# OCR-D/ocrd_keraslm

Measured on AMD Instinct MI355X. Metric: chars/sec training (stacked-LSTM forward+backward+Adam), higher is better.
Workload: dtype bf16; 1 GPU; cfg2: depth=2 width=512 length=256 V=256 1 context, stateful training, 3072 streams/GPU, synthetic 10M-char corpus (SURVEY.md 8d); streams_per_gpu=3072, global_batch=3072, seq_len=256, parallelism=dp1

## Files before the change

### include/keraslm_hip.h

```cpp
#ifndef KERASLM_HIP_H
#define KERASLM_HIP_H

#include <stddef.h>
#include <stdint.h>

#ifdef __cplusplus
extern "C" {
#endif

#define KL_ABI_VERSION 1

enum {
  KL_OK = 0,
  KL_ERR_SHAPE = 1,
  KL_ERR_LAUNCH = 2,
  KL_ERR_STATE = 3,
  KL_ERR_WORKSPACE = 4,
  KL_ERR_ARG = 5
};

#define KL_PREC_BF16 1
#define KL_PREC_SPLIT 3

typedef struct kl_config {
  int32_t depth;
  int32_t width;
  int32_t voc_size;
  int32_t n_ctx;
  int32_t ctx_vocab;
  int32_t ctx_dim;
} kl_config;

typedef struct kl_handle kl_handle;

int kl_abi_version(void);
const char* kl_error_string(int code);

size_t kl_param_count(const kl_config* cfg);
int kl_param_layout(const kl_config* cfg, int index, char* name, size_t name_cap, size_t* offset, size_t* rows,
                    size_t* cols);

kl_handle* kl_create(const kl_config* cfg);
void kl_destroy(kl_handle* h);

size_t kl_derived_bytes(const kl_handle* h);
int kl_bind(kl_handle* h, float* params , void* derived , size_t derived_bytes);

int kl_prepare(kl_handle* h, int precision, void* stream);

size_t kl_window_workspace_bytes(const kl_handle* h, int B, int T, int training);

int kl_set_window_mode(kl_handle* h, int last_only);

int kl_set_loss_rows(kl_handle* h, int rows);

int kl_forward_window(kl_handle* h, int B, int T, const int32_t* idx, const int32_t* ctx, const int32_t* tgt,
                      float* states, float* probs, float* loss_acc, void* ws, size_t ws_bytes, void* stream);

int kl_train_window(kl_handle* h, int B, int T, const int32_t* idx, const int32_t* ctx, const int32_t* tgt,
                    float* states, const float* dropout_masks, float* grads, float* loss_acc, void* ws,
                    size_t ws_bytes, void* stream);

int kl_adam_step(kl_handle* h, const float* grads, float* m, float* v, int t, float lr, float b1, float b2,
                 float eps, float clip, void* stream);
int kl_adam_step_scaled(kl_handle* h, const float* grads, float grad_scale, float* m, float* v, int t, float lr,
                        float b1, float b2, float eps, float clip, void* stream);

size_t kl_step_workspace_bytes(const kl_handle* h, int n);
int kl_step_batch(kl_handle* h, int n, const int32_t* idx, const int32_t* ctx, float* pool, const int32_t* slot_in,
                  const int32_t* slot_out, float* probs, void* ws, size_t ws_bytes, void* stream);

void* kl_host_alloc(size_t bytes);
void kl_host_free(void* p);
size_t kl_step_host_workspace_bytes(const kl_handle* h, int n);
int kl_step_batch_host(kl_handle* h, int n, const int32_t* idx, const int32_t* ctx, const int32_t* slot_in,
                       const int32_t* slot_out, const int32_t* target, float* pool, int head_k, float* probs_host,
                       float* heads_host, uint32_t* done_host, uint32_t ticket, void* ws, size_t ws_bytes, void* stream);
int kl_step_wait(const uint32_t* done_host, uint32_t ticket, double timeout_s);

int kl_state_dist2(const kl_handle* h, int n, const float* pool, const int32_t* a, const int32_t* b, int k,
                   float* out, void* stream);

int kl_trace_enable(kl_handle* h, int on);
int kl_trace_read(kl_handle* h, int kind, int* n_launches, float* total_ms, int* persistent,
                  double* flops_per_launch);
const char* kl_trace_kernel_name(kl_handle* h, int kind);

int kl_test_gemm_tn(const uint16_t* A, const uint16_t* B, void* C, const float* bias, int M, int N, int K, long lda,
                    long ldb, long ldc, int out_mode, int splits, void* stream);
int kl_test_gemm_an(const uint16_t* A_km, const uint16_t* B, float* C, int M, int N, int K, long lda_km, long ldb,
                    long ldc, int c_transposed, int b_km, void* stream);
int kl_test_thin_gemm(const float* A, long lda, const uint16_t* WT_hi, const uint16_t* WT_lo, long ldw, int M, int N,
                      int K, float* C, long ldc, int split, void* stream);

#ifdef __cplusplus
}
#endif
#endif
```

### ocrd_keraslm_amd/csrc/api.hip

```cpp
#include <hip/hip_runtime.h>
#include <stdio.h>
#include <stdlib.h>
#include <string.h>
#include <time.h>

#include <functional>
#include <utility>

#include <vector>

#include "kl_common.h"
#include "kl_kernels.h"

namespace {

inline size_t align_up(size_t x, size_t a) { return (x + a - 1) / a * a; }
inline int round_up_i(int x, int a) { return (x + a - 1) / a * a; }

struct Carver {
  unsigned char* base;
  size_t off = 0;
  explicit Carver(void* b) : base(reinterpret_cast<unsigned char*>(b)) {}
  template <typename T>
  T* take(size_t count) {
// ... 1749 lines not shown
    int e = 0;
    for (int l = 0; l < L && e == 0; ++l) {
      KlIncCellArgs a;
      memset(&a, 0, sizeof(a));
      a.n = n; a.W = W; a.split = split;
      a.pool = pool; a.slot_ld = slot_ld;
      a.h_off = 2 * l * W; a.c_off = (2 * l + 1) * W; a.x_off = l > 0 ? 2 * (l - 1) * W : -1;
      a.UF = d.UF[l]; a.KF = d.KF[l];
      a.bias = P + h->off_b[l];
      if (l == 0) {
        a.T1 = d.EK; a.i1 = dev_idx; a.T2 = d.CtxK[0]; a.i2 = dev_idx;
      }
      e = kl_launch_inc_cell(a, s, &hx, l == 0 ? dev_idx : nullptr);
      if (e == KL_ERR_SHAPE && l > 0) return e;
    }
    if (e == 0) {
      KlOperand op;
      memset(&op, 0, sizeof(op));
      op.A = pool + (size_t)2 * (L - 1) * W; op.lda = slot_ld; op.row_index = dev_idx; op.a_is_f32 = 1;
      op.WT_hi = d.E_hi; op.WT_lo = split == 3 ? d.E_lo : nullptr; op.ldw = W; op.K = W;
      KL_TRY(kl_launch_thin_gemm(&op, n, V, logits, V, nullptr, split, s));
      f.softmax = 1; f.slot_out = dev_idx;
      return kl_launch_step_finish(f, target ? &tx : nullptr, s);
    }
    if (e != KL_ERR_SHAPE) return e;
  }
  {
    const int Cc = C > 0 ? C : 1;
    std::vector<int32_t>& pk = h->host_pack;
    pk.resize((size_t)n * (4 + Cc));
    memcpy(pk.data(), idx, (size_t)n * 4);
    memcpy(pk.data() + n, slot_in, (size_t)n * 4);
    memcpy(pk.data() + 2 * (size_t)n, slot_out, (size_t)n * 4);
    if (target) memcpy(pk.data() + 3 * (size_t)n, target, (size_t)n * 4);
    else memset(pk.data() + 3 * (size_t)n, 0, (size_t)n * 4);
    if (C > 0) memcpy(pk.data() + 4 * (size_t)n, ctx, (size_t)n * C * 4);
    if (hipMemcpyAsync(dev_idx, pk.data(), pk.size() * 4, hipMemcpyHostToDevice, s) != hipSuccess) return KL_ERR_LAUNCH;
    KL_TRY(kl_step_batch(h, n, dev_idx, C > 0 ? dev_idx + 4 * (size_t)n : nullptr, pool, dev_idx + n, dev_idx + 2 * (size_t)n, logits,
                         rest, rest_bytes, stream));
    f.softmax = 0; f.slot_out = dev_idx + 2 * (size_t)n;
    f.target = target ? dev_idx + 3 * (size_t)n : nullptr;
    return kl_launch_step_finish(f, nullptr, s);
  }
}

int kl_step_wait(const uint32_t* done_host, uint32_t ticket, double timeout_s) {
  if (!done_host) return KL_ERR_ARG;
  const volatile uint32_t* flag = done_host;
  struct timespec t0;
  clock_gettime(CLOCK_MONOTONIC, &t0);
  for (unsigned spins = 0;; ++spins) {
    if (__atomic_load_n(flag, __ATOMIC_ACQUIRE) == ticket) return 0;
    __builtin_ia32_pause();
    if ((spins & 0x3ff) == 0x3ff) {
      struct timespec t1;
      clock_gettime(CLOCK_MONOTONIC, &t1);
      if ((double)(t1.tv_sec - t0.tv_sec) + 1e-9 * (double)(t1.tv_nsec - t0.tv_nsec) > timeout_s) {
        return hipGetLastError() == hipSuccess ? KL_ERR_STATE : KL_ERR_LAUNCH;
      }
    }
  }
}

int kl_state_dist2(const kl_handle* h, int n, const float* pool, const int32_t* a, const int32_t* b, int k, float* out,
                   void* stream) {
  if (!h || !pool || !a || !b || !out || n < 1) return KL_ERR_ARG;
  if (k < 0 || k >= 2 * h->cfg.depth) return KL_ERR_ARG;
  const int W = h->cfg.width;
  hipLaunchKernelGGL(state_dist2_kernel, dim3((n + 3) / 4), dim3(256), 0, (hipStream_t)stream, pool,
                     (long)2 * h->cfg.depth * W, W, k, a, b, n, out);
  return hip_ok(hipGetLastError());
}

int kl_test_gemm_tn(const uint16_t* A, const uint16_t* B, void* C, const float* bias, int M, int N, int K, long lda,
                    long ldb, long ldc, int out_mode, int splits, void* stream) {
  return kl_launch_gemm_tn(A, B, C, bias, M, N, K, lda, ldb, ldc, out_mode, splits, 1.f, (hipStream_t)stream);
}

int kl_test_gemm_an(const uint16_t* A_km, const uint16_t* B, float* C, int M, int N, int K, long lda_km, long ldb,
                    long ldc, int c_transposed, int b_km, void* stream) {
  return kl_launch_gemm_an(A_km, B, C, M, N, K, lda_km, ldb, ldc, c_transposed, (hipStream_t)stream, b_km);
}

int kl_test_thin_gemm(const float* A, long lda, const uint16_t* WT_hi, const uint16_t* WT_lo, long ldw, int M, int N,
                      int K, float* C, long ldc, int split, void* stream) {
  KlOperand op;
  memset(&op, 0, sizeof(op));
  op.A = A; op.lda = lda; op.a_is_f32 = 1; op.WT_hi = WT_hi; op.WT_lo = WT_lo; op.ldw = ldw; op.K = K;
  return kl_launch_thin_gemm(&op, M, N, C, ldc, nullptr, split, (hipStream_t)stream);
}

}

extern "C" int kl_test_fwd_step(const uint16_t* A, long lda, const uint16_t* WT, long ldw, int K, int n_ops,
                                int n_rows, int W, int fused, int iters, float* c_out, uint16_t* h_out,
                                void* stream) {
  KlFwdStep st[4];
  if (fused < 1 || fused > 4 || n_ops < 1 || n_ops > 2) return KL_ERR_ARG;
  for (int f = 0; f < fused; ++f) {
    KlFwdStep& S = st[f];
    memset(&S, 0, sizeof(S));
    S.n_rows = n_rows; S.W = W; S.split = 1; S.n_ops = n_ops;
    for (int p = 0; p < n_ops; ++p) {
      KlOperand& o = S.op[p];
      o.A = A; o.lda = lda; o.WT_hi = WT + (size_t)(f * 2 + p) * (size_t)4 * W * ldw; o.ldw = ldw;
      o.K = K; o.a_is_f32 = 0;
    }
    S.c_out = c_out + (size_t)f * n_rows * W; S.c_out_ld = W;
    S.h_out_bf16 = h_out + (size_t)f * n_rows * W; S.h_out_bf16_ld = W;
  }
  for (int i = 0; i < iters; ++i) {
    int e = kl_launch_fwd_steps(st, fused, (hipStream_t)stream);
    if (e) return e;
  }
  return 0;
}


namespace {

int run_graphed(kl_handle* h, const kl_handle::GraphKey& key, hipStream_t s, const std::function<int()>& body) {
  if (!h->graphs_enabled || h->trace_on || s == nullptr) return body();
  for (auto& g : h->graphs)
    if (g.first == key) return hip_ok(hipGraphLaunch(g.second, s));
  if (hipStreamBeginCapture(s, hipStreamCaptureModeThreadLocal) != hipSuccess) {
    (void)hipGetLastError();
    h->graphs_enabled = false;
    return body();
  }
  const int e = body();
  hipGraph_t graph = nullptr;
  const hipError_t ce = hipStreamEndCapture(s, &graph);
  if (e != 0 || ce != hipSuccess || graph == nullptr) {
    if (graph) (void)hipGraphDestroy(graph);
    (void)hipGetLastError();
    h->graphs_enabled = false;
    return e != 0 ? e : body();
  }
  hipGraphExec_t exec = nullptr;
  const hipError_t ie = hipGraphInstantiate(&exec, graph, nullptr, nullptr, 0);
  (void)hipGraphDestroy(graph);
  if (ie != hipSuccess || exec == nullptr) {
    (void)hipGetLastError();
    h->graphs_enabled = false;
    return body();
  }
  if (h->graphs.size() >= 16) h->drop_graphs();
  h->graphs.emplace_back(key, exec);
  return hip_ok(hipGraphLaunch(exec, s));
}

}

extern "C" int kl_set_loss_rows(kl_handle* h, int rows) {
  if (!h || rows < 0) return KL_ERR_ARG;
  h->loss_rows = rows;
  return 0;
}

extern "C" int kl_set_window_mode(kl_handle* h, int last_only) {
  if (!h) return KL_ERR_ARG;
  h->last_only = last_only ? 1 : 0;
  return 0;
}

extern "C" int kl_forward_window(kl_handle* h, int B, int T, const int32_t* idx, const int32_t* ctx, const int32_t* tgt,
// ... 83 lines not shown
```

### ocrd_keraslm_amd/csrc/gemm.hip

```cpp
#include <stdlib.h>
#include <string.h>

#include "kl_common.h"
#include "kl_kernels.h"

namespace {

constexpr int BN = 128, BK = 64;
constexpr int NTHREADS = 256;

__device__ __forceinline__ int lds_off(int row, int chunk) {
  return row * 128 + ((chunk ^ ((row >> 1) & 7)) << 4);
}

template <int OUT, int BM>
__global__ __launch_bounds__(NTHREADS) void gemm_tn_kernel(
    const bf16_t* __restrict__ A, const bf16_t* __restrict__ B, void* __restrict__ Cv,
    const float* __restrict__ bias, int M, int N, int K, long lda, long ldb, long ldc,
    int k_per_split, float alpha) {
  constexpr int WM = BM / 64;
  constexpr int WN = 4 / WM;
  constexpr int NT = BN / WN / 16;
  constexpr int ALOADS = BM * 8 / NTHREADS;
  extern __shared__ __attribute__((aligned(16))) unsigned char smem[];
// ... 574 lines not shown
        fa[i].u = *reinterpret_cast<const uint4*>(a_base + lds_off(wm * WROWS + i * 16 + fr, s * 4 + fq));
#pragma unroll
      for (int j = 0; j < NT; ++j)
        fb[j].u = *reinterpret_cast<const uint4*>(b_base + lds_off(wn * WCOLS + j * 16 + fr, s * 4 + fq));
      if (more) issue_half(nstage, s);
      __builtin_amdgcn_s_setprio(1);
#pragma unroll
      for (int i = 0; i < RF; ++i)
#pragma unroll
        for (int j = 0; j < NT; ++j) acc[i][j] = mfma16(fa[i].v, fb[j].v, acc[i][j]);
      __builtin_amdgcn_s_setprio(0);
    }
    stage = stage + 1 < LSTAGES ? stage + 1 : 0;
    if (++kt_c == nkt) {
      const int L = first + it_c * (int)gridDim.x;
      const int m0 = (L / tiles_n) * TBM, n0 = (L % tiles_n) * LBN;
      const int esz = out_bf16 ? 2 : 4;
      const long bytes = ((long)(M - m0 - 1) * ldc + (N - n0)) * esz;
      const __amdgpu_buffer_rsrc_t rsC = __builtin_amdgcn_make_buffer_rsrc(
          reinterpret_cast<char*>(C) + ((long)m0 * ldc + n0) * esz, 0, (int)(unsigned)(bytes > 0xffffffffL ? 0xffffffffL : bytes), 0x00020000);
      const int k = fr & 3, c4 = fr & ~3;
#pragma unroll
      for (int i = 0; i < RF; ++i) {
#pragma unroll
        for (int j = 0; j < NT; ++j) {
          f32x4 v = acc[i][j];
          quad_transpose(v, k);
          const int row = wm * WROWS + i * 16 + fq * 4 + k;
          const int col = wn * WCOLS + j * 16 + c4;
          f32x4 bv = f32x4{0.f, 0.f, 0.f, 0.f};
          if (bias != nullptr && n0 + col + 3 < N) bv = *reinterpret_cast<const f32x4*>(bias_l + n0 + col);
          v = v * alpha + bv;
          const unsigned off = (n0 + col < N) ? (unsigned)(((long)row * ldc + col) * esz) : 0xfffffff0u;
          if (out_bf16) {
            typedef __attribute__((ext_vector_type(2))) unsigned int u32x2g;
            const u32x2g pk = u32x2g{(unsigned)f2bf(v[0]) | ((unsigned)f2bf(v[1]) << 16), (unsigned)f2bf(v[2]) | ((unsigned)f2bf(v[3]) << 16)};
            __builtin_amdgcn_raw_buffer_store_b64(pk, rsC, (int)off, 0, 0);
          } else {
            __builtin_amdgcn_raw_buffer_store_b128(__builtin_bit_cast(u32x4g, v), rsC, (int)off, 0, 0);
          }
          acc[i][j] = f32x4{0.f, 0.f, 0.f, 0.f};
        }
      }
      kt_c = 0;
      ++it_c;
      stored = 2;
    }
  }
}

template <int RF, int WM, int WN>
int launch_long_t(int out_mode, dim3 grid, hipStream_t stream, const bf16_t* A, const bf16_t* B, void* C, const float* bias,
                  int M, int N, int K, long lda, long ldb, long ldc, int k_per_split, float alpha,
                  const KlGateEpi* gate = nullptr) {
  KlGateEpi epi;
  if (gate) epi = *gate;
  else memset(&epi, 0, sizeof(epi));
  const size_t lds = (size_t)LSTAGES * (16 * RF * WM + LBN) * 128;
  static const bool ilv = !(getenv("KL_GEMM_ILV") && getenv("KL_GEMM_ILV")[0] == '0');
  static const int remap = !(getenv("KL_GEMM_XCD") && getenv("KL_GEMM_XCD")[0] == '0');
#define KL_LONG_CASE(O)                                                                                                  \
  do {                                                                                                                   \
    static KlLdsGrant grant_a, grant_b;                                                  \
    if (kl_grant_lds(grant_a, reinterpret_cast<const void*>(&gemm_tn_long_kernel<O, true, RF, WM, WN>), lds)) return KL_ERR_LAUNCH;  \
    if (kl_grant_lds(grant_b, reinterpret_cast<const void*>(&gemm_tn_long_kernel<O, false, RF, WM, WN>), lds)) return KL_ERR_LAUNCH; \
    if (ilv) hipLaunchKernelGGL((gemm_tn_long_kernel<O, true, RF, WM, WN>), grid, dim3(64 * WM * WN), lds, stream, A, B, C,  \
                                bias, M, N, K, lda, ldb, ldc, k_per_split, alpha, epi, remap, 0, KlGemmSecond{});                        \
    else hipLaunchKernelGGL((gemm_tn_long_kernel<O, false, RF, WM, WN>), grid, dim3(64 * WM * WN), lds, stream, A, B, C,     \
                            bias, M, N, K, lda, ldb, ldc, k_per_split, alpha, epi, remap, 0, KlGemmSecond{});                            \
  } while (0)
  if (out_mode == 0) KL_LONG_CASE(0);
  else if (out_mode == 1) KL_LONG_CASE(1);
  else if (out_mode == 3) KL_LONG_CASE(3);
  else KL_LONG_CASE(2);
#undef KL_LONG_CASE
  return 0;
}

int launch_long(int out_mode, dim3 grid, hipStream_t stream, const bf16_t* A, const bf16_t* B, void* C, const float* bias,
                int M, int N, int K, long lda, long ldb, long ldc, int k_per_split, float alpha) {
  return launch_long_t<4, 4, 2>(out_mode, grid, stream, A, B, C, bias, M, N, K, lda, ldb, ldc, k_per_split, alpha);
}

}

int kl_launch_gemm_tn(const bf16_t* A, const bf16_t* B, void* C, const float* bias, int M, int N, int K,
                      long lda, long ldb, long ldc, int out_mode, int splits, float alpha, hipStream_t stream) {
  if (M <= 0 || N <= 0 || K <= 0) return 0;
  if ((K & 7) || (lda & 7) || (ldb & 7)) return KL_ERR_SHAPE;
  if (splits < 1) splits = 1;
  if (out_mode != 2) splits = 1;
  static const int long_mode = getenv("KL_GEMM_LONG") ? atoi(getenv("KL_GEMM_LONG")) : 2;
  const bool long_ok = (K % BK) == 0 && lda < (1L << 22) && ldb < (1L << 22);
  if (long_mode >= 1 && long_ok && out_mode == 2 && K >= 8192) {
    const int tiles = ((M + LBM - 1) / LBM) * ((N + LBN - 1) / LBN);
    int sp = (256 + tiles - 1) / tiles;
    const int nk = K / BK;
    if (sp > nk / 16) sp = nk / 16;
    if (sp < 1) sp = 1;
    const int kps = ((nk + sp - 1) / sp) * BK;
    sp = (K + kps - 1) / kps;
    dim3 grid((N + LBN - 1) / LBN, (M + LBM - 1) / LBM, sp);
    const int e = launch_long(out_mode, grid, stream, A, B, C, bias, M, N, K, lda, ldb, ldc, kps, alpha);
    if (e != 0) return e;
    return hipGetLastError() == hipSuccess ? 0 : KL_ERR_LAUNCH;
  }
  static const bool small_all = getenv("KL_GEMM_SMALL_ALL") && getenv("KL_GEMM_SMALL_ALL")[0] == '1';
  static const bool pers = !(getenv("KL_GEMM_PERS") && getenv("KL_GEMM_PERS")[0] == '0');
  if (pers && !small_all && long_mode >= 2 && long_ok && (out_mode == 0 || out_mode == 1) && K >= 6 * BK && K <= 16 * BK && (N & 3) == 0 && (ldc & 3) == 0 &&
      ((size_t)C & 15) == 0 && (bias == nullptr || N <= 2048) &&
      (long)((M + LBM - 1) / LBM) * ((N + LBN - 1) / LBN) >= 512) {
    static int n_wg = 0;
    if (!n_wg) {
      int dev = 0;
      hipDeviceProp_t prop;
      n_wg = (hipGetDevice(&dev) == hipSuccess && hipGetDeviceProperties(&prop, dev) == hipSuccess && prop.multiProcessorCount >= 8)
                 ? (prop.multiProcessorCount & ~7) : 256;
    }
    const int tiles_n = (N + LBN - 1) / LBN, total = ((M + LBM - 1) / LBM) * tiles_n;
    const size_t lds = (size_t)LSTAGES * (LBM + LBN) * 128 + (bias ? (size_t)N * 4 : 0);
    static KlLdsGrant grant;
    if (kl_grant_lds(grant, reinterpret_cast<const void*>(&gemm_tn_pers_kernel), (size_t)LSTAGES * (LBM + LBN) * 128 + 2048 * 4)) return KL_ERR_LAUNCH;
    hipLaunchKernelGGL(gemm_tn_pers_kernel, dim3(n_wg), dim3(512), lds, stream, A, B, (float*)C, bias, M, N, K, lda, ldb, ldc,
                       alpha, tiles_n, total, out_mode == 1 ? 1 : 0);
    return hipGetLastError() == hipSuccess ? 0 : KL_ERR_LAUNCH;
  }
  if (!small_all && long_mode >= 2 && long_ok && splits == 1 && K >= 256 && (long)((M + LBM - 1) / LBM) * ((N + LBN - 1) / LBN) >= 256) {
    dim3 grid((N + LBN - 1) / LBN, (M + LBM - 1) / LBM, 1);
    const int e = launch_long(out_mode, grid, stream, A, B, C, bias, M, N, K, lda, ldb, ldc, K, alpha);
    if (e != 0) return e;
    return hipGetLastError() == hipSuccess ? 0 : KL_ERR_LAUNCH;
  }
  if (long_mode >= 2 && long_ok && splits == 1 && K >= 512 && M >= 256 &&
      (long)((M + 63) / 64) * ((N + LBN - 1) / LBN) >= 64) {
    dim3 grid((N + LBN - 1) / LBN, (M + 63) / 64, 1);
    const int e = launch_long_t<2, 2, 4>(out_mode, grid, stream, A, B, C, bias, M, N, K, lda, ldb, ldc, K, alpha);
    if (e != 0) return e;
    return hipGetLastError() == hipSuccess ? 0 : KL_ERR_LAUNCH;
  }
  int k_per_split = (K + splits - 1) / splits;
  k_per_split = ((k_per_split + BK - 1) / BK) * BK;
  splits = (K + k_per_split - 1) / k_per_split;
  const int nbx = (N + BN - 1) / BN;
  const bool small = (long)nbx * ((M + 127) / 128) * splits < 256 && M > 64;
  if (small) {
    dim3 grid(nbx, (M + 63) / 64, splits);
    launch_bm<64>(out_mode, grid, stream, A, B, C, bias, M, N, K, lda, ldb, ldc, k_per_split, alpha);
  } else {
    dim3 grid(nbx, (M + 127) / 128, splits);
    launch_bm<128>(out_mode, grid, stream, A, B, C, bias, M, N, K, lda, ldb, ldc, k_per_split, alpha);
  }
  return hipGetLastError() == hipSuccess ? 0 : KL_ERR_LAUNCH;
}

static int an_rows_per_split(int M, int n_all, int K, long ld_max) {
  if (M <= 0 || n_all <= 0 || K <= 0 || (M % LBM) || (K % BK)) return 0;
  const int tiles = (M / LBM) * ((n_all + LBN - 1) / LBN);
  int sp = (256 + tiles - 1) / tiles;
  const int nk = K / BK;
  if (sp > nk / 16) sp = nk / 16;
  if (sp < 1) sp = 1;
  int kps = ((nk + sp - 1) / sp) * BK;
  while ((long)kps * ld_max * 2 >= 0x7fffffffL && kps > BK) {
    ++sp;
    kps = ((nk + sp - 1) / sp) * BK;
  }
  return (long)kps * ld_max * 2 < 0x7fffffffL ? kps : 0;
}

bool kl_gemm_an_applicable(int M, int N, int K, long lda_km) {
  if (lda_km & 7) return false;
  return an_rows_per_split(M, N, K, lda_km) > 0;
}

int kl_launch_gemm_an2(const bf16_t* A_km, const bf16_t* B, float* C, int M, int N, int K, long lda_km, long ldb, long ldc,
                       int c_transposed, const bf16_t* B2, float* C2, int N2, long ldb2, long ldc2, int c_transposed2,
                       hipStream_t stream, int b_km) {
  if (M <= 0 || N <= 0 || K <= 0) return 0;
  if (B2 != nullptr && ((N % LBN) || N2 <= 0 || (ldb2 & 7) || (!b_km && ldb2 >= (1L << 22)))) return KL_ERR_SHAPE;
  const int n_all = B2 != nullptr ? N + N2 : N;
  if ((lda_km & 7) || (ldb & 7) || (!b_km && ldb >= (1L << 22))) return KL_ERR_SHAPE;
  long ld_max = lda_km;
  if (b_km && ldb > ld_max) ld_max = ldb;
  if (b_km && B2 != nullptr && ldb2 > ld_max) ld_max = ldb2;
  const int kps = an_rows_per_split(M, n_all, K, ld_max);
  if (kps <= 0) return KL_ERR_SHAPE;
  const int sp = (K + kps - 1) / kps;
  dim3 grid((n_all + LBN - 1) / LBN, M / LBM, sp);
  KlGateEpi epi;
  memset(&epi, 0, sizeof(epi));
  KlGemmSecond second;
  memset(&second, 0, sizeof(second));
  if (B2 != nullptr) {
    second.B = B2;
    second.C = C2;
    second.n_first = N;
    second.N = N2;
    second.ldb = ldb2;
    second.ldc = ldc2;
    second.c_transposed = c_transposed2;
  }
  const size_t lds = (size_t)LSTAGES * (LBM + LBN) * 128;
  static const int remap = !(getenv("KL_GEMM_XCD") && getenv("KL_GEMM_XCD")[0] == '0');
  static KlLdsGrant grant_a, grant_b;
  if (kl_grant_lds(grant_a, reinterpret_cast<const void*>(&gemm_tn_long_kernel<2, true, 4, 4, 2, true, false>), lds)) return KL_ERR_LAUNCH;
  if (kl_grant_lds(grant_b, reinterpret_cast<const void*>(&gemm_tn_long_kernel<2, true, 4, 4, 2, true, true>), lds)) return KL_ERR_LAUNCH;
  if (b_km)
    hipLaunchKernelGGL((gemm_tn_long_kernel<2, true, 4, 4, 2, true, true>), grid, dim3(512), lds, stream, A_km, B, (void*)C,
                       (const float*)nullptr, M, N, K, lda_km, ldb, ldc, kps, 1.f, epi, remap, c_transposed, second);
  else
    hipLaunchKernelGGL((gemm_tn_long_kernel<2, true, 4, 4, 2, true, false>), grid, dim3(512), lds, stream, A_km, B, (void*)C,
                       (const float*)nullptr, M, N, K, lda_km, ldb, ldc, kps, 1.f, epi, remap, c_transposed, second);
  return hipGetLastError() == hipSuccess ? 0 : KL_ERR_LAUNCH;
}

int kl_launch_gemm_an(const bf16_t* A_km, const bf16_t* B, float* C, int M, int N, int K, long lda_km, long ldb, long ldc,
                      int c_transposed, hipStream_t stream, int b_km) {
  return kl_launch_gemm_an2(A_km, B, C, M, N, K, lda_km, ldb, ldc, c_transposed, nullptr, nullptr, 0, 0, 0, 0, stream, b_km);
}

int kl_launch_gemm_gates(const bf16_t* A3, const bf16_t* WTperm, int n, int W, int Kc, long lda, const KlGateEpi* epi,
                         hipStream_t stream) {
  if (n < 1 || (W & 31) || (Kc % BK) != 0 || (lda & 7) || lda >= (1L << 22) || !epi) return KL_ERR_SHAPE;
  dim3 grid(4 * W / LBN, (n + 63) / 64, 1);
  const int e = launch_long_t<2, 2, 4>(3, grid, stream, A3, WTperm, nullptr, nullptr, n, 4 * W, Kc, lda, lda, 0, Kc, 1.f, epi);
  if (e != 0) return e;
  return hipGetLastError() == hipSuccess ? 0 : KL_ERR_LAUNCH;
}
```

### ocrd_keraslm_amd/csrc/kl_kernels.h

```cpp
#pragma once
#include <hip/hip_runtime.h>
#include <stdint.h>

#include "keraslm_hip.h"

typedef unsigned short bf16_t;

#include <atomic>
#include <mutex>
#define KL_MAX_DEVICES 64
struct KlLdsGrant {
  std::atomic<size_t> granted[KL_MAX_DEVICES];
  std::mutex slow;
};
static inline int kl_grant_lds(KlLdsGrant& g, const void* fn, size_t lds) {
  int dev = 0;
  if (hipGetDevice(&dev) != hipSuccess) return KL_ERR_LAUNCH;
  if (dev < 0 || dev >= KL_MAX_DEVICES)
    return hipFuncSetAttribute(fn, hipFuncAttributeMaxDynamicSharedMemorySize, (int)lds) == hipSuccess ? 0 : KL_ERR_LAUNCH;
  if (lds <= g.granted[dev].load(std::memory_order_acquire)) return 0;
  std::lock_guard<std::mutex> lock(g.slow);
  if (lds <= g.granted[dev].load(std::memory_order_relaxed)) return 0;
  if (hipFuncSetAttribute(fn, hipFuncAttributeMaxDynamicSharedMemorySize, (int)lds) != hipSuccess) return KL_ERR_LAUNCH;
  g.granted[dev].store(lds, std::memory_order_release);
  return 0;
}

struct KlGatherRec {
  const float* pool; long slot_ld; const int* slot_in;
  int n, W, nb;
  bf16_t* out[4];
};
int kl_launch_gather_recurrent(const KlGatherRec& a, int L, hipStream_t stream);
int kl_launch_permute_gate_rows(const bf16_t* src, bf16_t* dst, int W, long cols, hipStream_t stream);

struct KlGateEpi {
  const float* T1; const int* i1;
  const float* T2; const int* i2;
  const float* bias;
  const float* c_prev; long c_ld; const int* slot_in;
  float* c_out; float* h_out; long out_ld; const int* slot_out;
  bf16_t* xn; long ldn; int kn; int nbn;
  int W;
};
int kl_launch_gemm_gates(const bf16_t* A3, const bf16_t* WTperm, int n, int W, int Kc, long lda, const KlGateEpi* epi,
                         hipStream_t stream);

int kl_launch_gemm_tn(const bf16_t* A, const bf16_t* B, void* C, const float* bias, int M, int N, int K,
                      long lda, long ldb, long ldc, int out_mode, int splits, float alpha, hipStream_t stream);
bool kl_gemm_an_applicable(int M, int N, int K, long lda_km);
int kl_launch_gemm_an(const bf16_t* A_km, const bf16_t* B, float* C, int M, int N, int K, long lda_km, long ldb, long ldc,
                      int c_transposed, hipStream_t stream, int b_km = 0);
int kl_launch_gemm_an2(const bf16_t* A_km, const bf16_t* B, float* C, int M, int N, int K, long lda_km, long ldb, long ldc,
                       int c_transposed, const bf16_t* B2, float* C2, int N2, long ldb2, long ldc2, int c_transposed2,
                       hipStream_t stream, int b_km);

struct KlOperand {
  const void* A;
  long lda;
  const int* row_index;
  const bf16_t* WT_hi;
  const bf16_t* WT_lo;
  long ldw;
  int K;
  int a_is_f32;
};

struct KlFwdStep {
  KlOperand op[2];
  int n_ops;
  int n_rows, W;
  int split;
  const float* T1; const int* i1; long t1_ld;
  const float* T2; const int* i2; long t2_ld;
  const float* bias;
  const float* c_prev; long c_prev_ld; const int* c_prev_index;
  const int* out_index;
  float* c_out; long c_out_ld;
  float* h_out_f32; long h_out_f32_ld;
  bf16_t* h_out_bf16; long h_out_bf16_ld;
  bf16_t* gates_out; long gates_ld;
  const float* hmask; long hmask_ld;
  bf16_t* hd_out_bf16; long hd_out_ld;
};
int kl_launch_fwd_steps(const KlFwdStep* steps, int n_steps, hipStream_t stream);

struct KlBwdStep {
  KlOperand op[2];
  int n_ops;
  int n_rows, W;
  const float* op0_mask; long op0_mask_ld;
  const float* dh_in; long dh_in_ld;
  const float* dh_mask; long dh_mask_ld;
  const bf16_t* gates; long gates_ld;
  const float* c; long c_ld;
  const float* c_prev; long c_prev_ld;
  const float* dc_in; long dc_in_ld;
  float* dc_out; long dc_out_ld;
  bf16_t* dz_out; long dz_ld;
};
int kl_launch_bwd_steps(const KlBwdStep* steps, int n_steps, hipStream_t stream);
int kl_zero_page_ready();

#define KL_SCAN_MAXL 4
struct KlScanFwd {
  int B, T, W, L;
  int n_rb, n_rg;
  const bf16_t* UT[KL_SCAN_MAXL];
  const bf16_t* KT[KL_SCAN_MAXL];
  const float* bias[KL_SCAN_MAXL];
  const float* P1;
  bf16_t* H[KL_SCAN_MAXL];
  float* C[KL_SCAN_MAXL];
  bf16_t* G[KL_SCAN_MAXL];
  bf16_t* Hd[KL_SCAN_MAXL];
  const float* mask[KL_SCAN_MAXL];
  unsigned* counters;
  unsigned* status;
  int sentinel;
  unsigned* xcc_slots; unsigned gen;
};
int kl_launch_scan_fwd(KlScanFwd args, hipStream_t stream);
bool kl_scan_w32_applicable(int B, int T, int W);
int kl_launch_scan_fwd_w32(KlScanFwd args, hipStream_t stream);

struct KlScanFwdSplit {
  int B, T, W, L;
  int n_rb, n_rg;
  const bf16_t* UT_hi[KL_SCAN_MAXL]; const bf16_t* UT_lo[KL_SCAN_MAXL];
  const bf16_t* KT_hi[KL_SCAN_MAXL]; const bf16_t* KT_lo[KL_SCAN_MAXL];
  const float* bias[KL_SCAN_MAXL];
  const float* P1;
  bf16_t* Xhi[KL_SCAN_MAXL]; bf16_t* Xlo[KL_SCAN_MAXL];
  float* Hf[KL_SCAN_MAXL];
  float* C[KL_SCAN_MAXL];
  unsigned* counters;
  unsigned* status;
  int sentinel;
// ... 177 lines not shown
```

### ocrd_keraslm_amd/lib/hipabi.py

```python
from __future__ import annotations

import ctypes as C
import os

_HERE = os.path.dirname(os.path.abspath(__file__))
LIB_PATH = os.environ.get("KL_LIB") or os.path.join(os.path.dirname(_HERE), "libkeraslm_hip.so")

KL_PREC_BF16 = 1
KL_PREC_SPLIT = 3


class KlConfig(C.Structure):
    _fields_ = [("depth", C.c_int32), ("width", C.c_int32), ("voc_size", C.c_int32),
                ("n_ctx", C.c_int32), ("ctx_vocab", C.c_int32), ("ctx_dim", C.c_int32)]


class KlError(RuntimeError):
    pass


SIGNATURES = {
    "kl_abi_version": (C.c_int, []),
    "kl_error_string": (C.c_char_p, [C.c_int]),
    "kl_param_count": (C.c_size_t, [C.POINTER(KlConfig)]),
    "kl_param_layout": (C.c_int, [C.POINTER(KlConfig), C.c_int, C.c_char_p, C.c_size_t,
                                  C.POINTER(C.c_size_t), C.POINTER(C.c_size_t), C.POINTER(C.c_size_t)]),
    "kl_create": (C.c_void_p, [C.POINTER(KlConfig)]),
    "kl_destroy": (None, [C.c_void_p]),
    "kl_derived_bytes": (C.c_size_t, [C.c_void_p]),
    "kl_bind": (C.c_int, [C.c_void_p, C.c_void_p, C.c_void_p, C.c_size_t]),
    "kl_prepare": (C.c_int, [C.c_void_p, C.c_int, C.c_void_p]),
    "kl_window_workspace_bytes": (C.c_size_t, [C.c_void_p, C.c_int, C.c_int, C.c_int]),
    "kl_forward_window": (C.c_int, [C.c_void_p, C.c_int, C.c_int, C.c_void_p, C.c_void_p, C.c_void_p, C.c_void_p,
                                    C.c_void_p, C.c_void_p, C.c_void_p, C.c_size_t, C.c_void_p]),
    "kl_train_window": (C.c_int, [C.c_void_p, C.c_int, C.c_int, C.c_void_p, C.c_void_p, C.c_void_p, C.c_void_p,
                                  C.c_void_p, C.c_void_p, C.c_void_p, C.c_void_p, C.c_size_t, C.c_void_p]),
    "kl_adam_step": (C.c_int, [C.c_void_p, C.c_void_p, C.c_void_p, C.c_void_p, C.c_int, C.c_float, C.c_float,
                               C.c_float, C.c_float, C.c_float, C.c_void_p]),
    "kl_adam_step_scaled": (C.c_int, [C.c_void_p, C.c_void_p, C.c_float, C.c_void_p, C.c_void_p, C.c_int, C.c_float, C.c_float,
                                     C.c_float, C.c_float, C.c_float, C.c_void_p]),
    "kl_step_workspace_bytes": (C.c_size_t, [C.c_void_p, C.c_int]),
    "kl_step_batch": (C.c_int, [C.c_void_p, C.c_int, C.c_void_p, C.c_void_p, C.c_void_p, C.c_void_p, C.c_void_p,
                                C.c_void_p, C.c_void_p, C.c_size_t, C.c_void_p]),
    "kl_host_alloc": (C.c_void_p, [C.c_size_t]),
    "kl_host_free": (None, [C.c_void_p]),
    "kl_step_host_workspace_bytes": (C.c_size_t, [C.c_void_p, C.c_int]),
    "kl_step_batch_host": (C.c_int, [C.c_void_p, C.c_int, C.c_void_p, C.c_void_p, C.c_void_p, C.c_void_p, C.c_void_p,
                                     C.c_void_p, C.c_int, C.c_void_p, C.c_void_p, C.c_void_p, C.c_uint32, C.c_void_p,
                                     C.c_size_t, C.c_void_p]),
    "kl_step_wait": (C.c_int, [C.c_void_p, C.c_uint32, C.c_double]),
    "kl_state_dist2": (C.c_int, [C.c_void_p, C.c_int, C.c_void_p, C.c_void_p, C.c_void_p, C.c_int, C.c_void_p,
                                 C.c_void_p]),
    "kl_trace_enable": (C.c_int, [C.c_void_p, C.c_int]),
    "kl_set_window_mode": (C.c_int, [C.c_void_p, C.c_int]),
    "kl_set_loss_rows": (C.c_int, [C.c_void_p, C.c_int]),
    "kl_trace_kernel_name": (C.c_char_p, [C.c_void_p, C.c_int]),
    "kl_trace_read": (C.c_int, [C.c_void_p, C.c_int, C.POINTER(C.c_int), C.POINTER(C.c_float), C.POINTER(C.c_int),
                                C.POINTER(C.c_double)]),
    "kl_test_gemm_tn": (C.c_int, [C.c_void_p, C.c_void_p, C.c_void_p, C.c_void_p, C.c_int, C.c_int, C.c_int,
                                  C.c_long, C.c_long, C.c_long, C.c_int, C.c_int, C.c_void_p]),
    "kl_test_gemm_an": (C.c_int, [C.c_void_p, C.c_void_p, C.c_void_p, C.c_int, C.c_int, C.c_int, C.c_long, C.c_long,
                                  C.c_long, C.c_int, C.c_int, C.c_void_p]),
    "kl_test_thin_gemm": (C.c_int, [C.c_void_p, C.c_long, C.c_void_p, C.c_void_p, C.c_long, C.c_int, C.c_int,
                                    C.c_int, C.c_void_p, C.c_long, C.c_int, C.c_void_p]),
}

_lib = None


def load():
    global _lib
    if _lib is not None:
        return _lib
    if not os.path.exists(LIB_PATH):
        raise KlError("HIP extension %s not built: run `make -C ocrd_keraslm_amd/csrc` "
                      "(the Rater has no CPU fallback)" % LIB_PATH)
    lib = C.CDLL(LIB_PATH)
    for name, (res, args) in SIGNATURES.items():
        fn = getattr(lib, name)
        fn.restype = res
        fn.argtypes = args
    _lib = lib
    return lib


def check(code, what=""):
    if code != 0:
        msg = load().kl_error_string(code).decode()
        raise KlError("%s failed: %s (code %d)" % (what or "keraslm_hip call", msg, code))
```

Before: 33.92 million chars/s.

## Add 256x256 multi-stage wide GEMM kernel for weight-gradient accumulation

Adds a new 512-thread GEMM kernel for the A-transposed weight-gradient path. It uses 256x256 output tiles, a 4-5 stage LDS ring fed by direct global-to-LDS buffer loads, transposed LDS reads, and split-K atomic accumulation. By default it replaces the long-tile kernel whenever a second operand is present and B is K-major. The aim is more data reuse per tile and deeper prefetch for the large weight-gradient GEMMs, at the cost of a single block per CU and more atomics from split-K.

```diff
diff --git a/include/keraslm_hip.h b/include/keraslm_hip.h
--- a/include/keraslm_hip.h
+++ b/include/keraslm_hip.h
@@ -90,6 +90,9 @@
                     long ldb, long ldc, int out_mode, int splits, void* stream);
 int kl_test_gemm_an(const uint16_t* A_km, const uint16_t* B, float* C, int M, int N, int K, long lda_km, long ldb,
                     long ldc, int c_transposed, int b_km, void* stream);
+int kl_test_gemm_wide(const uint16_t* A_km, const uint16_t* B, float* C, int M, int N, int K, long lda_km, long ldb,
+                      long ldc, int c_transposed, const uint16_t* B2, float* C2, int N2, long ldb2, long ldc2,
+                      int c_transposed2, int b_km, int tile, void* stream);
 int kl_test_thin_gemm(const float* A, long lda, const uint16_t* WT_hi, const uint16_t* WT_lo, long ldw, int M, int N,
                       int K, float* C, long ldc, int split, void* stream);
 
diff --git a/ocrd_keraslm_amd/csrc/api.hip b/ocrd_keraslm_amd/csrc/api.hip
--- a/ocrd_keraslm_amd/csrc/api.hip
+++ b/ocrd_keraslm_amd/csrc/api.hip
@@ -1855,6 +1855,13 @@
   return kl_launch_gemm_an(A_km, B, C, M, N, K, lda_km, ldb, ldc, c_transposed, (hipStream_t)stream, b_km);
 }
 
+int kl_test_gemm_wide(const uint16_t* A_km, const uint16_t* B, float* C, int M, int N, int K, long lda_km, long ldb,
+                      long ldc, int c_transposed, const uint16_t* B2, float* C2, int N2, long ldb2, long ldc2,
+                      int c_transposed2, int b_km, int tile, void* stream) {
+  return kl_test_gemm_an_tile(A_km, B, C, M, N, K, lda_km, ldb, ldc, c_transposed, B2, C2, N2, ldb2, ldc2, c_transposed2,
+                              b_km, tile, (hipStream_t)stream);
+}
+
 int kl_test_thin_gemm(const float* A, long lda, const uint16_t* WT_hi, const uint16_t* WT_lo, long ldw, int M, int N,
                       int K, float* C, long ldc, int split, void* stream) {
   KlOperand op;
diff --git a/ocrd_keraslm_amd/csrc/gemm.hip b/ocrd_keraslm_amd/csrc/gemm.hip
--- a/ocrd_keraslm_amd/csrc/gemm.hip
+++ b/ocrd_keraslm_amd/csrc/gemm.hip
@@ -680,6 +680,201 @@
   return launch_long_t<4, 4, 2>(out_mode, grid, stream, A, B, C, bias, M, N, K, lda, ldb, ldc, k_per_split, alpha);
 }
 
+#ifndef KL_GEMM_WIDE_STAGES
+#define KL_GEMM_WIDE_STAGES 4
+#endif
+constexpr int WBM = 256, WBN = 256, WBK = 32;
+constexpr int WSTAGE_BYTES = (WBM + WBN) * WBK * 2;
+
+__device__ __forceinline__ int wide_rm_swz(int n) {
+  const int g = (n >> 2) & 3;
+  return g ^ ((g & 1) << 1);
+}
+
+template <bool BTR, int NS>
+__global__ __launch_bounds__(512, 1) void gemm_an_wide_kernel(
+    const bf16_t* __restrict__ A, const bf16_t* __restrict__ B_, float* __restrict__ C_, int M, int N_, int K, long lda,
+    long ldb_, long ldc_, int k_per_split, int xcd_remap, int c_t_, const KlGemmSecond second) {
+  constexpr int WN = 4, RF = 8, NT = 4;
+  constexpr int WROWS = 16 * RF, WCOLS = 16 * NT;
+  constexpr int NP = 4;
+  static_assert(NS >= 3 && NS <= 5, "ring depth");
+  const bf16_t* __restrict__ B = B_;
+  float* __restrict__ Cv = C_;
+  int N = N_, c_t = c_t_;
+  long ldb = ldb_, ldc = ldc_;
+  extern __shared__ __attribute__((aligned(16))) unsigned char smem[];
+  const int tid = threadIdx.x;
+  const int lane = tid & 63;
+  const int wave = __builtin_amdgcn_readfirstlane(tid >> 6);
+  const int wm = wave / WN, wn = wave % WN;
+  int bx = blockIdx.x, by = blockIdx.y, bz = blockIdx.z;
+  {
+    const unsigned nx = gridDim.x, ny = gridDim.y, total = nx * ny * gridDim.z;
+    if (xcd_remap && (total & 7) == 0) {
+      const unsigned lin = bx + nx * (by + ny * bz);
+      const unsigned re = (lin & 7) * (total >> 3) + (lin >> 3);
+      bx = re % nx;
+      by = (re / nx) % ny;
+      bz = re / (nx * ny);
+    }
+  }
+  const int m0 = by * WBM;
+  int n0 = bx * WBN;
+  if (second.B != nullptr) {
+    if (n0 >= second.n_first) {
+      n0 -= second.n_first;
+      B = second.B;
+      Cv = reinterpret_cast<float*>(second.C);
+      N = second.N;
+      ldb = second.ldb;
+      ldc = second.ldc;
+      c_t = second.c_transposed;
+    } else {
+      N = second.n_first;
+    }
+  }
+  const int kbeg = bz * k_per_split;
+  const int kend = min(K, kbeg + k_per_split);
+  const int nkt = (kend - kbeg) / WBK;
+
+  auto clamp31 = [](long v) { return (int)(v > 0x7fffffffL ? 0x7fffffffL : (v < 0 ? 0 : v)); };
+  const __amdgpu_buffer_rsrc_t rsA = __builtin_amdgcn_make_buffer_rsrc(
+      const_cast<bf16_t*>(A + (long)kbeg * lda + m0), 0, clamp31(((long)(kend - kbeg - 1) * lda + (M - m0)) * 2), 0x00020000);
+  const __amdgpu_buffer_rsrc_t rsB = BTR
+      ? __builtin_amdgcn_make_buffer_rsrc(const_cast<bf16_t*>(B + (long)kbeg * ldb + n0), 0, clamp31(((long)(kend - kbeg - 1) * ldb + (N - n0)) * 2), 0x00020000)
+      : __builtin_amdgcn_make_buffer_rsrc(const_cast<bf16_t*>(B + (long)n0 * ldb), 0, clamp31(((long)(N - n0 - 1) * ldb + K) * 2), 0x00020000);
+  unsigned vo[NP];
+#pragma unroll
+  for (int j = 0; j < NP; ++j) {
+    const int p = 2 * wave + (j & 1);
+    if (j < 2 || BTR) {
+      const int krow = 2 * p + (lane >> 5);
+      const int c = (lane & 31) ^ (2 * ((krow & 3) | (((krow >> 3) & 1) << 2)));
+      vo[j] = (unsigned)((long)krow * (j < 2 ? lda : ldb) * 2 + c * 16);
+    } else {
+      const int row = 16 * p + (lane >> 2);
+      const int c = (lane & 3) ^ wide_rm_swz(row);
+      vo[j] = (unsigned)((long)row * ldb * 2 + c * 16);
+    }
+  }
+  const unsigned lds0 = (unsigned)(size_t)(lds_void_t*)smem;
+  auto issue_half = [&](int kt, int stage, int half) {
+    const int soff_a = (int)((long)kt * WBK * lda * 2);
+    const int soff_b = BTR ? (int)((long)kt * WBK * ldb * 2) : (kbeg + kt * WBK) * 2;
+    const unsigned sbase = lds0 + stage * WSTAGE_BYTES + (2 * wave + half) * 1024;
+    glds16(rsA, vo[half], soff_a, sbase);
+    glds16(rsB, vo[2 + half], soff_b, sbase + WBM * WBK * 2);
+  };
+
+  f32x4 acc[RF][NT];
+#pragma unroll
+  for (int i = 0; i < RF; ++i)
+#pragma unroll
+    for (int j = 0; j < NT; ++j) acc[i][j] = f32x4{0.f, 0.f, 0.f, 0.f};
+
+  const int fr = lane & 15, fq = lane >> 4;
+  const int q = fr >> 2, pp = fr & 3;
+  const int fl = 2 * (q | ((fq & 1) << 2));
+  const unsigned tr_lane = (unsigned)((fq * 8 + q) * 512 + (pp >> 1) * 16 + 8 * (pp & 1));
+  auto tr_frag = [&](const unsigned char* base, int col0) {
+    const unsigned char* p = base + tr_lane + (((col0 >> 3) ^ fl) * 16);
+    const s16x4 lo = __builtin_amdgcn_ds_read_tr16_b64_v4i16((lds_s16x4*)(p));
+    const s16x4 hi = __builtin_amdgcn_ds_read_tr16_b64_v4i16((lds_s16x4*)(p + 4 * 512));
+    frag16 f;
+    f.s[0] = (bf16_t)lo.x; f.s[1] = (bf16_t)lo.y; f.s[2] = (bf16_t)lo.z; f.s[3] = (bf16_t)lo.w;
+    f.s[4] = (bf16_t)hi.x; f.s[5] = (bf16_t)hi.y; f.s[6] = (bf16_t)hi.z; f.s[7] = (bf16_t)hi.w;
+    return f;
+  };
+  auto read_first = [&](int st, frag16* fb, frag16* fa) {
+    const unsigned char* a_base = smem + st * WSTAGE_BYTES;
+    const unsigned char* b_base = a_base + WBM * WBK * 2;
+#pragma unroll
+    for (int j = 0; j < NT; ++j) {
+      if (BTR) {
+        fb[j] = tr_frag(b_base, wn * WCOLS + j * 16);
+      } else {
+        const int n = wn * WCOLS + j * 16 + fr;
+        fb[j].u = *reinterpret_cast<const uint4*>(b_base + n * 64 + ((fq ^ wide_rm_swz(n)) << 4));
+      }
+    }
+#pragma unroll
+    for (int i = 0; i < RF / 2; ++i) fa[i] = tr_frag(a_base, wm * WROWS + i * 16);
+  };
+  auto wait_steps = [&](int n) {
+    if (NS > 4 && n >= 4) asm volatile("s_waitcnt vmcnt(%0)" ::"n"(4 * NP) : "memory");
+    else if (n >= 3) asm volatile("s_waitcnt vmcnt(%0)" ::"n"(3 * NP) : "memory");
+    else if (n == 2) asm volatile("s_waitcnt vmcnt(%0)" ::"n"(2 * NP) : "memory");
+    else if (n == 1) asm volatile("s_waitcnt vmcnt(%0)" ::"n"(NP) : "memory");
+    else asm volatile("s_waitcnt vmcnt(0)" ::: "memory");
+  };
+
+#pragma unroll
+  for (int d = 0; d < NS; ++d)
+    if (d < nkt) {
+      issue_half(d, d, 0);
+      issue_half(d, d, 1);
+    }
+  frag16 fb0[NT], fl0[RF / 2], fb1[NT], fl1[RF / 2], fh[RF / 2];
+  if (nkt > 0) {
+    wait_steps(min(NS - 1, nkt - 1));
+    __builtin_amdgcn_s_barrier();
+    read_first(0, fb0, fl0);
+  }
+  auto kstep = [&](int kt, int stage, frag16* fb, frag16* fl, frag16* fbn, frag16* fln) {
+    const unsigned char* a_base = smem + stage * WSTAGE_BYTES;
+#pragma unroll
+    for (int i = 0; i < RF / 2; ++i) fh[i] = tr_frag(a_base, wm * WROWS + (RF / 2 + i) * 16);
+    __builtin_amdgcn_s_setprio(1);
+#pragma unroll
+    for (int i = 0; i < RF / 2; ++i)
+#pragma unroll
+      for (int j = 0; j < NT; ++j) acc[i][j] = mfma16(fl[i].v, fb[j].v, acc[i][j]);
+    __builtin_amdgcn_s_setprio(0);
+    if (kt + 1 < nkt) {
+      asm volatile("s_waitcnt lgkmcnt(0)" ::: "memory");
+      wait_steps(min(NS - 2, nkt - 2 - kt));
+      __builtin_amdgcn_s_barrier();
+      if (kt + NS < nkt) {
+        issue_half(kt + NS, stage, 0);
+        issue_half(kt + NS, stage, 1);
+      }
+      read_first(stage + 1 < NS ? stage + 1 : 0, fbn, fln);
+    }
+    __builtin_amdgcn_s_setprio(1);
+#pragma unroll
+    for (int i = 0; i < RF / 2; ++i)
+#pragma unroll
+      for (int j = 0; j < NT; ++j) acc[RF / 2 + i][j] = mfma16(fh[i].v, fb[j].v, acc[RF / 2 + i][j]);
+    __builtin_amdgcn_s_setprio(0);
+  };
+  int stage = 0;
+  for (int kt = 0; kt < nkt; kt += 2) {
+    kstep(kt, stage, fb0, fl0, fb1, fl1);
+    stage = stage + 1 < NS ? stage + 1 : 0;
+    if (kt + 1 < nkt) {
+      kstep(kt + 1, stage, fb1, fl1, fb0, fl0);
+      stage = stage + 1 < NS ? stage + 1 : 0;
+    }
+  }
+
+#pragma unroll
+  for (int i = 0; i < RF; ++i) {
+#pragma unroll
+    for (int j = 0; j < NT; ++j) {
+      const int col = n0 + wn * WCOLS + j * 16 + fr;
+      if (col >= N) continue;
+#pragma unroll
+      for (int r = 0; r < 4; ++r) {
+        const int row = m0 + wm * WROWS + i * 16 + fq * 4 + r;
+        if (row >= M) continue;
+        if (c_t) atomicAdd(Cv + (long)col * ldc + row, acc[i][j][r]);
+        else atomicAdd(Cv + (long)row * ldc + col, acc[i][j][r]);
+      }
+    }
+  }
+}
+
 }
 
 int kl_launch_gemm_tn(const bf16_t* A, const bf16_t* B, void* C, const float* bias, int M, int N, int K,
@@ -771,22 +966,41 @@
   return an_rows_per_split(M, N, K, lda_km) > 0;
 }
 
-int kl_launch_gemm_an2(const bf16_t* A_km, const bf16_t* B, float* C, int M, int N, int K, long lda_km, long ldb, long ldc,
-                       int c_transposed, const bf16_t* B2, float* C2, int N2, long ldb2, long ldc2, int c_transposed2,
-                       hipStream_t stream, int b_km) {
+static int an_wide_rows_per_split(int M, int n_tiles, int K, long ld_max) {
+  if (M <= 0 || n_tiles <= 0 || K <= 0 || (M % WBM) || (K % WBK)) return 0;
+  const int tiles = (M / WBM) * n_tiles;
+  int sp = (256 + tiles - 1) / tiles;
+  const int nk = K / WBK;
+  if (sp > nk / 16) sp = nk / 16;
+  if (sp < 1) sp = 1;
+  int kps = ((nk + sp - 1) / sp) * WBK;
+  while ((long)kps * ld_max * 2 >= 0x7fffffffL && kps > WBK) {
+    ++sp;
+    kps = ((nk + sp - 1) / sp) * WBK;
+  }
+  return (long)kps * ld_max * 2 < 0x7fffffffL ? kps : 0;
+}
+
+template <bool BTR, int NS>
+static int launch_an_wide(dim3 grid, hipStream_t stream, const bf16_t* A_km, const bf16_t* B, float* C, int M, int N, int K,
+                          long lda_km, long ldb, long ldc, int kps, int remap, int c_transposed, const KlGemmSecond& second) {
+  const size_t lds = (size_t)NS * WSTAGE_BYTES;
+  static KlLdsGrant grant;
+  if (kl_grant_lds(grant, reinterpret_cast<const void*>(&gemm_an_wide_kernel<BTR, NS>), lds)) return KL_ERR_LAUNCH;
+  hipLaunchKernelGGL((gemm_an_wide_kernel<BTR, NS>), grid, dim3(512), lds, stream, A_km, B, C, M, N, K, lda_km, ldb, ldc, kps,
+                     remap, c_transposed, second);
+  return hipGetLastError() == hipSuccess ? 0 : KL_ERR_LAUNCH;
+}
+
+static int gemm_an2_tile(const bf16_t* A_km, const bf16_t* B, float* C, int M, int N, int K, long lda_km, long ldb, long ldc,
+                         int c_transposed, const bf16_t* B2, float* C2, int N2, long ldb2, long ldc2, int c_transposed2,
+                         hipStream_t stream, int b_km, int tile) {
   if (M <= 0 || N <= 0 || K <= 0) return 0;
-  if (B2 != nullptr && ((N % LBN) || N2 <= 0 || (ldb2 & 7) || (!b_km && ldb2 >= (1L << 22)))) return KL_ERR_SHAPE;
-  const int n_all = B2 != nullptr ? N + N2 : N;
+  if (B2 != nullptr && (N2 <= 0 || (ldb2 & 7) || (!b_km && ldb2 >= (1L << 22)))) return KL_ERR_SHAPE;
   if ((lda_km & 7) || (ldb & 7) || (!b_km && ldb >= (1L << 22))) return KL_ERR_SHAPE;
   long ld_max = lda_km;
   if (b_km && ldb > ld_max) ld_max = ldb;
   if (b_km && B2 != nullptr && ldb2 > ld_max) ld_max = ldb2;
-  const int kps = an_rows_per_split(M, n_all, K, ld_max);
-  if (kps <= 0) return KL_ERR_SHAPE;
-  const int sp = (K + kps - 1) / kps;
-  dim3 grid((n_all + LBN - 1) / LBN, M / LBM, sp);
-  KlGateEpi epi;
-  memset(&epi, 0, sizeof(epi));
   KlGemmSecond second;
   memset(&second, 0, sizeof(second));
   if (B2 != nullptr) {
@@ -798,8 +1012,29 @@
     second.ldc = ldc2;
     second.c_transposed = c_transposed2;
   }
+  static const int remap = !(getenv("KL_GEMM_XCD") && getenv("KL_GEMM_XCD")[0] == '0');
+  static const bool wide_on = !(getenv("KL_GEMM_WIDE") && getenv("KL_GEMM_WIDE")[0] == '0');
+  const int wide_ntiles = B2 != nullptr ? ((N % WBN) ? 0 : N / WBN + (N2 + WBN - 1) / WBN) : (N + WBN - 1) / WBN;
+  const int wide_kps = wide_ntiles > 0 ? an_wide_rows_per_split(M, wide_ntiles, K, ld_max) : 0;
+  if (tile < 0) tile = (wide_on && wide_kps > 0 && B2 != nullptr && b_km) ? KL_GEMM_WIDE_STAGES : 0;
+  if (tile != 0) {
+    if (wide_kps <= 0 || (tile != 4 && tile != 5)) return KL_ERR_SHAPE;
+    dim3 grid(wide_ntiles, M / WBM, (K + wide_kps - 1) / wide_kps);
+    if (tile == 4)
+      return b_km ? launch_an_wide<true, 4>(grid, stream, A_km, B, C, M, N, K, lda_km, ldb, ldc, wide_kps, remap, c_transposed, second)
+                  : launch_an_wide<false, 4>(grid, stream, A_km, B, C, M, N, K, lda_km, ldb, ldc, wide_kps, remap, c_transposed, second);
+    return b_km ? launch_an_wide<true, 5>(grid, stream, A_km, B, C, M, N, K, lda_km, ldb, ldc, wide_kps, remap, c_transposed, second)
+                : launch_an_wide<false, 5>(grid, stream, A_km, B, C, M, N, K, lda_km, ldb, ldc, wide_kps, remap, c_transposed, second);
+  }
+  if (B2 != nullptr && (N % LBN)) return KL_ERR_SHAPE;
+  const int n_all = B2 != nullptr ? N + N2 : N;
+  const int kps = an_rows_per_split(M, n_all, K, ld_max);
+  if (kps <= 0) return KL_ERR_SHAPE;
+  const int sp = (K + kps - 1) / kps;
+  dim3 grid((n_all + LBN - 1) / LBN, M / LBM, sp);
+  KlGateEpi epi;
+  memset(&epi, 0, sizeof(epi));
   const size_t lds = (size_t)LSTAGES * (LBM + LBN) * 128;
-  static const int remap = !(getenv("KL_GEMM_XCD") && getenv("KL_GEMM_XCD")[0] == '0');
   static KlLdsGrant grant_a, grant_b;
   if (kl_grant_lds(grant_a, reinterpret_cast<const void*>(&gemm_tn_long_kernel<2, true, 4, 4, 2, true, false>), lds)) return KL_ERR_LAUNCH;
   if (kl_grant_lds(grant_b, reinterpret_cast<const void*>(&gemm_tn_long_kernel<2, true, 4, 4, 2, true, true>), lds)) return KL_ERR_LAUNCH;
@@ -812,6 +1047,18 @@
   return hipGetLastError() == hipSuccess ? 0 : KL_ERR_LAUNCH;
 }
 
+int kl_launch_gemm_an2(const bf16_t* A_km, const bf16_t* B, float* C, int M, int N, int K, long lda_km, long ldb, long ldc,
+                       int c_transposed, const bf16_t* B2, float* C2, int N2, long ldb2, long ldc2, int c_transposed2,
+                       hipStream_t stream, int b_km) {
+  return gemm_an2_tile(A_km, B, C, M, N, K, lda_km, ldb, ldc, c_transposed, B2, C2, N2, ldb2, ldc2, c_transposed2, stream, b_km, -1);
+}
+
+int kl_test_gemm_an_tile(const bf16_t* A_km, const bf16_t* B, float* C, int M, int N, int K, long lda_km, long ldb, long ldc,
+                         int c_transposed, const bf16_t* B2, float* C2, int N2, long ldb2, long ldc2, int c_transposed2,
+                         int b_km, int tile, hipStream_t stream) {
+  return gemm_an2_tile(A_km, B, C, M, N, K, lda_km, ldb, ldc, c_transposed, B2, C2, N2, ldb2, ldc2, c_transposed2, stream, b_km, tile);
+}
+
 int kl_launch_gemm_an(const bf16_t* A_km, const bf16_t* B, float* C, int M, int N, int K, long lda_km, long ldb, long ldc,
                       int c_transposed, hipStream_t stream, int b_km) {
   return kl_launch_gemm_an2(A_km, B, C, M, N, K, lda_km, ldb, ldc, c_transposed, nullptr, nullptr, 0, 0, 0, 0, stream, b_km);
diff --git a/ocrd_keraslm_amd/csrc/kl_kernels.h b/ocrd_keraslm_amd/csrc/kl_kernels.h
--- a/ocrd_keraslm_amd/csrc/kl_kernels.h
+++ b/ocrd_keraslm_amd/csrc/kl_kernels.h
@@ -54,6 +54,9 @@
 int kl_launch_gemm_an2(const bf16_t* A_km, const bf16_t* B, float* C, int M, int N, int K, long lda_km, long ldb, long ldc,
                        int c_transposed, const bf16_t* B2, float* C2, int N2, long ldb2, long ldc2, int c_transposed2,
                        hipStream_t stream, int b_km);
+int kl_test_gemm_an_tile(const bf16_t* A_km, const bf16_t* B, float* C, int M, int N, int K, long lda_km, long ldb, long ldc,
+                         int c_transposed, const bf16_t* B2, float* C2, int N2, long ldb2, long ldc2, int c_transposed2,
+                         int b_km, int tile, hipStream_t stream);
 
 struct KlOperand {
   const void* A;
diff --git a/ocrd_keraslm_amd/lib/hipabi.py b/ocrd_keraslm_amd/lib/hipabi.py
--- a/ocrd_keraslm_amd/lib/hipabi.py
+++ b/ocrd_keraslm_amd/lib/hipabi.py
@@ -61,6 +61,9 @@
                                   C.c_long, C.c_long, C.c_long, C.c_int, C.c_int, C.c_void_p]),
     "kl_test_gemm_an": (C.c_int, [C.c_void_p, C.c_void_p, C.c_void_p, C.c_int, C.c_int, C.c_int, C.c_long, C.c_long,
                                   C.c_long, C.c_int, C.c_int, C.c_void_p]),
+    "kl_test_gemm_wide": (C.c_int, [C.c_void_p, C.c_void_p, C.c_void_p, C.c_int, C.c_int, C.c_int, C.c_long, C.c_long,
+                                    C.c_long, C.c_int, C.c_void_p, C.c_void_p, C.c_int, C.c_long, C.c_long, C.c_int,
+                                    C.c_int, C.c_int, C.c_void_p]),
     "kl_test_thin_gemm": (C.c_int, [C.c_void_p, C.c_long, C.c_void_p, C.c_void_p, C.c_long, C.c_int, C.c_int,
                                     C.c_int, C.c_void_p, C.c_long, C.c_int, C.c_void_p]),
 }
```

Result: no change. 34.04 million chars/s, median of 6 (+0.4%).
